# mapillary/OpenSfM

Hardware: AMD Instinct MI355X
Metric: image-pairs matched/sec (+ BA LM-iters/sec, 5k cams / 500k pts) (higher is better)
Workload: dtype i8 (exact int32 accumulate) + f64 RANSAC

## Files before the change

### opensfm_amd/csrc/ba.hip

```cpp
#ifdef OSFM_HIPEMU
#include <cassert>
#endif
#include <chrono>
#include <cmath>
#include <cstdio>
#include <cstring>
#include <numeric>
#include <vector>

#include <rocprim/rocprim.hpp>

#include "ba_math.h"
#include "osfm_internal.h"

using namespace osfm_ba;

namespace {

constexpr int kCoopObs = 256;

typedef double osfm_v2d __attribute__((ext_vector_type(2)));
__device__ __forceinline__ void st2(double *p, double a, double b) {
  osfm_v2d v;
  v.x = a;
// ... 126 lines not shown
    for (int m = 32; m >= 1; m >>= 1) v[k] += __shfl_xor(v[k], m);
  const int lane = threadIdx.x & 63, w = threadIdx.x >> 6;
  const int nw = (blockDim.x + 63) >> 6;
  if (nw == 1) return;
  if (lane == 0)
#pragma unroll
    for (int k = 0; k < NV; k++) lds[w * NV + k] = v[k];
  __syncthreads();
  if (threadIdx.x == 0)
#pragma unroll
    for (int k = 0; k < NV; k++) {
      double s = lds[k];
      for (int w2 = 1; w2 < nw; w2++) s += lds[w2 * NV + k];
      v[k] = s;
    }
}

template <int NV, int W, int N>
__device__ __forceinline__ void shot_sum(double (&v)[NV], double (&lds)[N] ) {
  static_assert(W == 1 || N >= W * NV, "shot_sum: lds is shorter than NV doubles per wavefront");
#ifdef OSFM_HIPEMU
  assert((int)blockDim.x == 64 * W);
#endif
#pragma unroll
  for (int i = 0; i < NV; i++)
#pragma unroll
    for (int m = 32; m >= 1; m >>= 1) v[i] += __shfl_xor(v[i], m);
  if (W == 1) return;
  const int lane = threadIdx.x & 63, w = threadIdx.x >> 6;
  if (lane == 0)
// ... 108 lines not shown
  double *qD;
  double *qE[2];
  double *qX;
  double *qXt;
  double *qx, *qy;
  int qT;
  double *qP, *qR, *qRn, *qC;
  double *zc;
  double *y;
  double *x, *r, *z, *p, *Ap, *b;
  double *scal;
  double *partial;
  double *partial2;
  double *dotp;
  double *rrp;
  int gen;
  GenDev g;
};

#define JA(o, c) d.Jpm[(long)(c) * d.M + (o)]
constexpr int kRowComps = 17;
constexpr int R_JP = 2, R_JR = 8, R_U = 14, R_V = 15, R_WT = 16;

__device__ __forceinline__ void row_jk(const Dev &d, long o, int s, double (&jk)[6]) {
  const int ci = d.shot_camera[s];
  const double u = JA(o, R_U), v = JA(o, R_V), wt = JA(o, R_WT), sg = d.o_sigma[o];
  const double *cam = d.cams + 3 * ci;
  const double k1 = cam[0], k2 = cam[1], f = cam[2];
  const bool other = d.cam_model && d.cam_model[ci] >= 2;
  double J[6];
// ... 186 lines not shown
__device__ __forceinline__ void up_residual(const Dev &d, int s, double r[3], double J[9]) {
  const double *R = d.shotR + 36 * (long)s, *u = d.up + 3 * (long)s;
  const double isd = 1.0 / d.up_sigma[s];
#pragma unroll
  for (int i = 0; i < 3; i++) {
    const double z = R[i] * u[0] + R[3 + i] * u[1] + R[6 + i] * u[2];
    r[i] = isd * (z - (i == 2 ? 1.0 : 0.0));
#pragma unroll
    for (int k = 0; k < 3; k++) {
      const double *dR = R + 9 + 9 * k;
      J[3 * i + k] = -isd * (dR[i] * u[0] + dR[3 + i] * u[1] + dR[6 + i] * u[2]);
    }
  }
}

__global__ void __launch_bounds__(1024) prior_cost_kernel(Dev d, const double *cams, const double *poses, const double *partial, long npart, double *out, double *absmax_slot, int jac) {
  __shared__ double lds[64];
  for (int c = 0; c < 2; c++) {
    double v[1] = {0.0};
    for (long i = threadIdx.x; i < npart; i += blockDim.x) v[0] += partial[i * 2 + c];
    block_sum<1, 1024>(v, lds);
    if (threadIdx.x == 0) out[c] = v[0];
    __syncthreads();
  }
  if (threadIdx.x == 0 && absmax_slot) *absmax_slot = 0.0;
  double v[1] = {0.0};
  for (int c = threadIdx.x; c < d.NC; c += blockDim.x) {
    if (d.cam_fixed[c]) continue;
    const double *q = cams + 3 * c, *pr = d.cam_prior + 3 * c, *sg = d.cam_sigma + 3 * c;
    const double e0 = (q[0] - pr[0]) / fmax(sg[0], kEps), e1 = (q[1] - pr[1]) / fmax(sg[1], kEps);
    const double e2 = log(q[2] / pr[2]) / fmax(sg[2], kEps);
    v[0] += 0.5 * (e0 * e0 + e1 * e1 + e2 * e2);
  }
  if (d.gps && d.gps_sigma)
    for (int s = threadIdx.x; s < d.S; s += blockDim.x) {
      const double sg = d.gps_sigma[s];
      const bool fixed = d.shot_fixed && d.shot_fixed[s];
      const double p3[3] = {poses[6 * s + 3], poses[6 * s + 4], poses[6 * s + 5]}, g3[3] = {d.gps[3 * s], d.gps[3 * s + 1], d.gps[3 * s + 2]};
      if (!(sg > 0) || fixed) continue;
      for (int i = 0; i < 3; i++) {
        const double e = (p3[i] - g3[i]) / sg;
        v[0] += 0.5 * e * e;
      }
    }
  if (d.up && d.up_sigma)
    for (int s = threadIdx.x; s < d.S; s += blockDim.x) {
      if (!(d.up_sigma[s] > 0) || (d.shot_fixed && d.shot_fixed[s])) continue;
      double r[3], J[9], rho, rho1;
      up_residual(d, s, r, J);
      loss_eval(OSFM_LOSS_CAUCHY, 1.0, r[0] * r[0] + r[1] * r[1] + r[2] * r[2], rho, rho1);
      v[0] += 0.5 * rho;
      if (jac) {
        const double wt = sqrt(rho1);
        for (int i = 0; i < 3; i++) d.up_r[3 * s + i] = wt * r[i];
        for (int i = 0; i < 9; i++) d.up_J[9 * s + i] = wt * J[i];
      }
    }
  block_sum<1, 1024>(v, lds);
  if (threadIdx.x == 0) out[0] += v[0];
}

template <int W>
__global__ void __launch_bounds__(64 * W) shot_grad_kernel(Dev d, const double *poses, int loss, double la) {
  __shared__ double red[W > 1 ? W * 36 : 1];
  const int s = (int)xcd_contiguous(blockIdx.x, gridDim.x), lane = threadIdx.x;
  const ShotFrame f = shot_frame(d, s);
  double v[36];
#pragma unroll
  for (int i = 0; i < 36; i++) v[i] = 0;
  for (long k = d.shot_off[s] + lane; k < d.shot_off[s + 1]; k += 64 * W) {
    double r[2], Jp[6], Jc[12], Jk[6];
    const int p = d.sm_point[k];
    project_obs<true>(f.model, d.pts + 3 * (long)p, f.pose, f.R, f.R + 9, f.cam, d.sm_x[k], d.sm_y[k], 1.0 / d.sm_sigma[k], r, Jp, Jc, Jk);
    double rho, rho1;
// ... 69 lines not shown
  const bool fixed = d.cam_fixed[c];
  const double *q = cams + 3 * c, *pr = d.cam_prior + 3 * c, *sg = d.cam_sigma + 3 * c;
  const double w0 = 1.0 / fmax(sg[0], kEps), w1 = 1.0 / fmax(sg[1], kEps), w2 = 1.0 / fmax(sg[2], kEps);
  const double e[3] = {(q[0] - pr[0]) * w0, (q[1] - pr[1]) * w1, log(q[2] / pr[2]) * w2};
  const double j[3] = {w0, w1, w2 / q[2]};
  const int dg[3] = {3, 5, 8};
  for (int k = 0; k < 3; k++) {
    const int i = d.cam0 + 3 * c + k;
    d.g_red[i] = fixed ? 0.0 : v[k] + j[k] * e[k];
    d.prior_diag[i] = fixed ? 0.0 : j[k] * j[k];
    d.diag_red[i] = fixed ? 0.0 : v[dg[k]] + j[k] * j[k];
  }
  for (int i = 0; i < 6; i++) d.Hcc[21 * (long)d.S + 6 * c + i] = v[3 + i];
}

constexpr int kCamRedT = 1024;
__global__ void __launch_bounds__(kCamRedT) cam_reduce_kernel(Dev d, int ncomp, const double *grad_cams) {
  __shared__ double lds[16 * 9];
  const int c = blockIdx.x;
  double v[9] = {0, 0, 0, 0, 0, 0, 0, 0, 0};
  for (int s0 = threadIdx.x; s0 < d.S; s0 += 4 * kCamRedT) {
    double p[4][9];
    bool on[4];
#pragma unroll
    for (int u = 0; u < 4; u++) {
      const int s = s0 + u * kCamRedT;
      const bool in = s < d.S;
      on[u] = in && d.shot_camera[in ? s : 0] == c;
#pragma unroll
      for (int i = 0; i < 9; i++) p[u][i] = (in && i < ncomp) ? d.part[9 * (long)s + i] : 0.0;
    }
#pragma unroll
    for (int u = 0; u < 4; u++)
      if (on[u])
#pragma unroll
        for (int i = 0; i < 9; i++) v[i] += p[u][i];
  }
  block_sum<9, kCamRedT>(v, lds);
  if (threadIdx.x == 0) {
    for (int i = 0; i < ncomp; i++) d.camred[9 * c + i] = v[i];
    if (grad_cams) cam_grad_one(d, grad_cams, c, v);
  }
}

__global__ void cam_grad_kernel(Dev d, const double *cams) {
  const int c = blockIdx.x * blockDim.x + threadIdx.x;
  if (c >= d.NC) return;
  double v[9];
  for (int i = 0; i < 9; i++) v[i] = d.camred[9 * c + i];
  cam_grad_one(d, cams, c, v);
}

__global__ void scale_init_kernel(Dev d) {
  const long i = (long)blockIdx.x * blockDim.x + threadIdx.x;
  if (i < d.nred) {
    bool fixed;
// ... 2291 lines not shown

__global__ void dot2_kernel(const double *a, const double *b, const double *c, const double *e, int n, double *o0, double *o1) {
  __shared__ double lds[32];
  double v[2] = {0, 0};
#pragma unroll 4
  for (int i = threadIdx.x; i < n; i += blockDim.x) {
    v[0] += a[i] * b[i];
    if (c) v[1] += c[i] * e[i];
  }
  block_sum<2, 1024>(v, lds);
  if (threadIdx.x == 0) {
    *o0 = v[0];
    if (c) *o1 = v[1];
  }
}
__global__ void pcg_init_kernel(const double *b, const double *z, double *x, double *r, double *p, int n, double *o_rz, double *o_bb, const double *sc, double *y) {
  __shared__ double lds[32];
  double v[2] = {0, 0};
#pragma unroll 4
  for (int i = threadIdx.x; i < n; i += blockDim.x) {
    const double bi = b[i], zi = z[i];
    x[i] = 0.0;
    r[i] = bi;
    p[i] = zi;
    y[i] = sc[i] * zi;
    v[0] += bi * zi;
    v[1] += bi * bi;
  }
  block_sum<2, 1024>(v, lds);
  if (threadIdx.x == 0) {
    *o_rz = v[0];
    *o_bb = v[1];
  }
}
__global__ void __launch_bounds__(TPB) pcg_step1_kernel(double *x, double *r, const double *p, const double *Ap, int n, const double *rz, const double *dot_part, int nparts,
                                                         double *o_pAp, double *rr_part, const double *sc = nullptr, double *y_out = nullptr) {
  __shared__ double lds[32];
  __shared__ double s_alpha;
  const int i = blockIdx.x * blockDim.x + threadIdx.x;
  {
    double pAp;
    if (dot_part) {
      double a[1] = {0.0};
      for (int q = threadIdx.x; q < nparts; q += TPB) a[0] += dot_part[q];
      block_sum<1, TPB>(a, lds);
      pAp = a[0];
    } else
// ... 29 lines not shown
  } else if (b < d.S + d.NC) {
    const int c = b - d.S;
    const double *Bi = d.Binv + 36 * (long)d.S + 9 * c, *rr = r + d.cam0 + 3 * c;
    for (int i = 0; i < 3; i++) z[d.cam0 + 3 * c + i] = Bi[3 * i] * rr[0] + Bi[3 * i + 1] * rr[1] + Bi[3 * i + 2] * rr[2];
  }
}
__global__ void pcg_step2_kernel(double *p, const double *z, int n, const double *rz_old, const double *rz_new, const double *sc, double *y) {
  const int i = blockIdx.x * blockDim.x + threadIdx.x;
  if (i >= n) return;
  const double beta = *rz_old != 0.0 ? *rz_new / *rz_old : 0.0;
  const double pi = z[i] + beta * p[i];
  p[i] = pi;
  y[i] = sc[i] * pi;
}

__global__ void __launch_bounds__(1024) candidate_kernel(Dev d, const double *y, const double *partial, long npart, double *out, const double *part2, long npart2,
                                                         double *out2, int do_rot) {
  __shared__ double lds[16 * 3];
  {
    double m[1] = {0.0};
    for (long i = threadIdx.x; i < npart; i += blockDim.x) m[0] += partial[i];
    block_sum<1, 1024>(m, lds);
    if (threadIdx.x == 0) out[0] = m[0];
    __syncthreads();
  }
  for (int c = 0; c < 2; c++) {
    double m[1] = {0.0};
    for (long i = threadIdx.x; i < npart2; i += blockDim.x) m[0] += part2[2 * i + c];
    block_sum<1, 1024>(m, lds);
    if (threadIdx.x == 0) out2[c] = m[0];
    __syncthreads();
  }
  double v[3] = {0, 0, 0};
  for (int c = threadIdx.x; c < d.NC; c += blockDim.x) {
    const double *q = d.cams + 3 * c;
    const bool fixed = d.cam_fixed[c];
    if (!fixed) {
      const double *pr = d.cam_prior + 3 * c, *sg = d.cam_sigma + 3 * c;
      const double wq[3] = {1.0 / fmax(sg[0], kEps), 1.0 / fmax(sg[1], kEps), 1.0 / fmax(sg[2], kEps)};
      const double e[3] = {(q[0] - pr[0]) * wq[0], (q[1] - pr[1]) * wq[1], log(q[2] / pr[2]) * wq[2]};
      const double j[3] = {wq[0], wq[1], wq[2] / q[2]};
      for (int k = 0; k < 3; k++) {
        const double m = j[k] * y[d.cam0 + 3 * c + k];
        v[0] -= m * (e[k] + 0.5 * m);
      }
    }
    for (int k = 0; k < 3; k++) {
      const double dl = fixed ? 0.0 : y[d.cam0 + 3 * c + k];
      d.cams_n[3 * c + k] = q[k] + dl;
      if (!fixed) {
        v[1] += dl * dl;
        v[2] += q[k] * q[k];
      }
    }
  }
  for (int s = threadIdx.x; s < d.S; s += blockDim.x) {
    const bool fixed = d.shot_fixed && d.shot_fixed[s];
    double ys[6], ps[6], g3[3] = {0, 0, 0}, sg = 0.0;
#pragma unroll
    for (int k = 0; k < 6; k++) {
      ys[k] = y[6 * s + k];
      ps[k] = d.poses[6 * s + k];
    }
    if (d.gps && d.gps_sigma) {
      sg = d.gps_sigma[s];
#pragma unroll
      for (int k = 0; k < 3; k++) g3[k] = d.gps[3 * s + k];
    }
    if (!fixed && sg > 0) {
      const double wq = 1.0 / sg;
      for (int k = 0; k < 3; k++) {
// ... 9 lines not shown
        v[0] -= m * (ru[i] + 0.5 * m);
      }
    }
    double pn[6];
    for (int k = 0; k < 6; k++) {
      const double dl = fixed ? 0.0 : ys[k];
      pn[k] = ps[k] + dl;
      d.poses_n[6 * s + k] = pn[k];
      if (!fixed) {
        v[1] += dl * dl;
        v[2] += ps[k] * ps[k];
      }
    }
    if (do_rot) rot_and_derivs(pn, d.shotR + 36 * (long)s, d.shotR + 36 * (long)s + 9);
  }
  block_sum<3, 1024>(v, lds);
  if (threadIdx.x == 0) {
    out[0] += v[0];
    out[1] = v[1];
    out[2] = v[2];
  }
}
__global__ void __launch_bounds__(TPB) candidate_points_kernel(Dev d, double *part) {
  __shared__ double lds[16];
  const long i = (long)blockIdx.x * TPB + threadIdx.x;
  double v[2] = {0, 0};
  if (i < 3L * d.P) {
    const bool fixed = d.point_fixed && d.point_fixed[i / 3];
    const double dl = fixed ? 0.0 : d.d_pt[i];
    d.pts_n[i] = d.pts[i] + dl;
    if (!fixed) {
      v[0] = dl * dl;
      v[1] = d.pts[i] * d.pts[i];
    }
  }
// ... 43 lines not shown
}
__global__ void reproj_kernel(Dev d, double *out) {
  const long o = (long)blockIdx.x * TPB + threadIdx.x;
  if (o >= d.M) return;
  const int s = d.o_shot[o], p = d.o_point[o];
  const double *R = d.shotR + 36 * (long)s;
  double r[2];
  const int cmodel = d.cam_model ? d.cam_model[d.shot_camera[s]] : 0;
  project_obs<false>(cmodel, d.pts + 3 * (long)p, d.poses + 6 * (long)s, R, R + 9,
                     cmodel >= 2 ? d.cam_ext + 16 * d.shot_camera[s] : d.cams + 3 * d.shot_camera[s], d.o_x[o], d.o_y[o],
                     1.0, r, nullptr, nullptr, nullptr);
  out[2 * o] = r[0];
  out[2 * o + 1] = r[1];
}

__global__ void border_dots_kernel(const double *Bc, const double *W, int nb, int n, double *out) {
  __shared__ double lds[32];
  const int i = blockIdx.x / nb, j = blockIdx.x % nb;
  double v[1] = {0.0};
#pragma unroll 4
  for (int t = threadIdx.x; t < n; t += blockDim.x) v[0] += Bc[(long)i * n + t] * W[(long)j * n + t];
  block_sum<1, 1024>(v, lds);
  if (threadIdx.x == 0) out[blockIdx.x] = v[0];
}
__global__ void border_rhs_kernel(const double *Bc, const double *SigInv, const double *r, double *z, int nb, int n, int cam0) {
  __shared__ double lds[32];
  __shared__ double y[8];
  for (int i = 0; i < nb; i++) {
    double v[1] = {0.0};
    for (int t = threadIdx.x; t < n; t += blockDim.x) v[0] += Bc[(long)i * n + t] * z[t];
    block_sum<1, 1024>(v, lds);
    if (threadIdx.x == 0) y[i] = r[cam0 + i] - v[0];
    __syncthreads();
  }
  if (threadIdx.x < nb) {
    double acc = 0.0;
    for (int j = 0; j < nb; j++) acc += SigInv[threadIdx.x * nb + j] * y[j];
    z[cam0 + threadIdx.x] = acc;
// ... 578 lines not shown
      }
      if (ctx->h_stage) {
        char *dst = (char *)ctx->h_stage + staged;
        memcpy(dst, h, bytes);
        staged += padded;
        e = hipMemcpyAsync(p, dst, bytes, hipMemcpyHostToDevice, st);
        return p;
      }
    }
    e = hipMemcpy(p, h, bytes, hipMemcpyHostToDevice);
    return p;
  }
};

inline int nblk(long n, int t = TPB) { return (int)std::max<long>(1, (n + t - 1) / t); }

struct BaSwitches {
  bool no_sband = getenv("OSFM_BA_NO_SBAND") != nullptr;
  bool check_band = getenv("OSFM_BA_CHECK_BAND") != nullptr;
  bool band_per_shot = getenv("OSFM_BA_BAND_PER_SHOT") != nullptr;
  bool wide_ldlt = getenv("OSFM_BA_WIDE_LDLT") != nullptr;
  const char *dense_cr_budget = getenv("OSFM_BA_DENSE_CR_BUDGET");
  bool gen_full_rows = getenv("OSFM_BA_GEN_FULL_ROWS") != nullptr;
  bool no_fast = getenv("OSFM_BA_NO_FAST") != nullptr;
  int fast_fail_at = getenv("OSFM_BA_FAST_FAIL_AT") ? atoi(getenv("OSFM_BA_FAST_FAIL_AT")) : -1;
  bool trace = getenv("OSFM_BA_TRACE") != nullptr;
  bool spin = getenv("OSFM_BA_NO_SPIN") == nullptr;
  double spin_us = getenv("OSFM_BA_SPIN_US") ? atof(getenv("OSFM_BA_SPIN_US")) : 2000.0;
};

// ... 156 lines not shown
    double *dh = (double *)dev_pinned;
    const int want = ++seq;
    hipLaunchKernelGGL(publish_kernel, dim3(1), dim3(64), 0, st, a, na, dh + ha_off, b, nb, (int *)(dh + 32) + hb_off, c, nc, dh + 34, (int *)(dh + 34 + nbr_), want);
    OSFM_HIP(hipGetLastError());
    const auto t0 = std::chrono::steady_clock::now();
    for (long it = 0; __atomic_load_n(hseq, __ATOMIC_ACQUIRE) != want; it++) {
      if ((it & 0x3FF) == 0x3FF && std::chrono::duration<double>(std::chrono::steady_clock::now() - t0).count() * 1e6 > spin_us) {
        OSFM_HIP(hipStreamSynchronize(st));
        OSFM_REQUIRE(__atomic_load_n(hseq, __ATOMIC_ACQUIRE) == want, OSFM_E_HIP, "the device never published round trip %d", want);
      }
    }
    return OSFM_OK;
  }

  void rot(const double *poses) { hipLaunchKernelGGL(shot_rot_kernel, dim3(nblk(d.S, 64)), dim3(64), 0, st, d, poses); }

  template <class F>
  void with_gen_model(F &&f) const {
    using std::integral_constant;
    if (d.g.NRr == 3) f(integral_constant<int, 3>{}, integral_constant<int, -1>{});
    else if (gen_uniform_model == OSFM_CAMERA_BROWN) f(integral_constant<int, 2>{}, integral_constant<int, OSFM_CAMERA_BROWN>{});
    else if (gen_uniform_model == OSFM_CAMERA_FISHEYE_OPENCV) f(integral_constant<int, 2>{}, integral_constant<int, OSFM_CAMERA_FISHEYE_OPENCV>{});
    else if (gen_uniform_model == OSFM_CAMERA_PERSPECTIVE) f(integral_constant<int, 2>{}, integral_constant<int, OSFM_CAMERA_PERSPECTIVE>{});
    else f(integral_constant<int, 2>{}, integral_constant<int, -1>{});
  }
  template <class F>
  void with_gen_kw(F &&f) const {
    using std::integral_constant;
    if (d.g.KW <= 4) f(integral_constant<int, 4>{});
    else if (d.g.KW <= 9) f(integral_constant<int, 9>{});
// ... 112 lines not shown
    if (!y_ready) hipLaunchKernelGGL(scale_vec_kernel, dim3(nblk(d.nred)), dim3(TPB), 0, sq, d.sc_red, x, d.y, d.nred);
    gen_rows_apply(0, sq);
    if (have_bpri && d.g.NB > 0) hipLaunchKernelGGL(gen_bpri_dot_kernel, dim3(d.g.NB, kBpriSlices), dim3(256), 0, sq, d, (const double *)d.y);
    hipLaunchKernelGGL(gen_schur_finish_kernel, dim3(nblk(d.nred)), dim3(TPB), 0, sq, d, x, (const double *)d.y, out, radius, 0, d.M > 0 ? 1 : 0,
                       have_bpri ? 1 : 0, dot_part);
  }

  void eval_enqueue(const double *cams, const double *poses, const double *pts, bool jac, bool rot_done = false) {
    if (d.gen) {
      const bool cand = poses == d.poses_n;
      return gen_eval_enqueue(cand ? d.g.cam_n : d.g.cam, cand ? d.g.bias_n : d.g.bias, cand ? d.g.rc_n : d.g.rc, poses, pts, jac);
    }
    if (!rot_done) rot(poses);
    if (jac) hipLaunchKernelGGL(eval_kernel<true>, dim3(d.nwg), dim3(kCoopObs), 0, st, d, cams, poses, pts, loss, loss_a);
    else hipLaunchKernelGGL(eval_kernel<false>, dim3(d.nwg), dim3(kCoopObs), 0, st, d, cams, poses, pts, loss, loss_a);
    hipLaunchKernelGGL(prior_cost_kernel, dim3(1), dim3(1024), 0, st, d, cams, poses, (const double *)d.partial, (long)d.nwg, d.scal + 8, d.scal + 10, jac ? 1 : 0);
  }
  int eval(const double *cams, const double *poses, const double *pts, bool jac, double *cost, double *sumsq) {
    eval_enqueue(cams, poses, pts, jac);
    OSFM_HIP(hipGetLastError());
    OSFM_TRY(fetch(d.scal + 8, 2, 0));
    *cost = hscal[0];
    if (sumsq) *sumsq = hscal[1];
    return OSFM_OK;
  }
  void gradients() {
    if (d.gen) return gen_gradients();
    if (shot_waves() > 1) hipLaunchKernelGGL(shot_grad_kernel<kShotWavesSmall>, dim3(d.S), dim3(64 * kShotWavesSmall), 0, st, d, (const double *)d.poses, loss, loss_a);
    else hipLaunchKernelGGL(shot_grad_kernel<1>, dim3(d.S), dim3(64), 0, st, d, (const double *)d.poses, loss, loss_a);
    if (!cams_inert) hipLaunchKernelGGL(cam_reduce_kernel, dim3(d.NC), dim3(kCamRedT), 0, st, d, 9, (const double *)d.cams);
    else hipLaunchKernelGGL(cam_grad_kernel, dim3(nblk(d.NC, 64)), dim3(64), 0, st, d, d.cams);
  }
  void bcr_solve_set(const RhsSet &rs) {
    if (use_sband) {
      hipLaunchKernelGGL(sband_solve_kernel, dim3((rs.nrhs + kSbSolveWaves - 1) / kSbSolveWaves), dim3(64 * kSbSolveWaves), sband_solve_lds(d.S, d.bw), st, d,
                         (const double *)sbL, rs, SbFuse{0, 0.0, nullptr, nullptr, nullptr, nullptr, nullptr, nullptr, nullptr});
      return;
    }
    const int N = d.ncl;
    const unsigned q = (unsigned)rs.nrhs;
    auto ne = [N](int s) { return (N + 2 * s - 1) / (2 * s); };
    int st0 = 2;
    while (ne(st0) > kMidWaves) st0 *= 2;
    hipLaunchKernelGGL(bcr_down_kernel, dim3(ne(1), q), dim3(64), 0, st, d, 1, rs, 1);
    for (int s = 2; s < st0; s *= 2) hipLaunchKernelGGL(bcr_down_kernel, dim3(ne(s), q), dim3(64), 0, st, d, s, rs, 0);
// ... 246 lines not shown
        if (shot_waves() > 1) hipLaunchKernelGGL((border_shot_kernel<3, kShotWavesSmall>), dim3(d.S), dim3(64 * kShotWavesSmall), 0, sx, d, wB, Bc, partB);
        else hipLaunchKernelGGL((border_shot_kernel<3, 1>), dim3(d.S), dim3(64), 0, sx, d, wB, Bc, partB);
        hipLaunchKernelGGL(border_cam_kernel<3>, dim3(d.NC), dim3(TPB), 0, sx, d, partB, dCm, radius);
      } else {
        hipLaunchKernelGGL(border_point_kernel<6>, dim3(d.nwg), dim3(kCoopObs), 0, sx, d, wB);
        if (shot_waves() > 1) hipLaunchKernelGGL((border_shot_kernel<6, kShotWavesSmall>), dim3(d.S), dim3(64 * kShotWavesSmall), 0, sx, d, wB, Bc, partB);
        else hipLaunchKernelGGL((border_shot_kernel<6, 1>), dim3(d.S), dim3(64), 0, sx, d, wB, Bc, partB);
        hipLaunchKernelGGL(border_cam_kernel<6>, dim3(d.NC), dim3(TPB), 0, sx, d, partB, dCm, radius);
      }
    }
    if (!pl.sband_fuse) rhs_enqueue(radius, sx);
    if (pl.side2) OSFM_HIP(hipEventRecord(ev_join, pl.side2));
    return OSFM_OK;
  }
  void border_sigma(int nb, int n6) {
    hipLaunchKernelGGL(border_dots_kernel, dim3(nb * nb), dim3(TPB), 0, st, Bc, Wb, nb, n6, dots);
    if (nb <= 6)
      hipLaunchKernelGGL(border_sigma_kernel, dim3(1), dim3(64), 0, st, dCm, dots, SigInv, nb, d_status + 1);
    else
      hipLaunchKernelGGL(gen_border_sigma_kernel, dim3(1), dim3(256), (size_t)nb * 2 * nb * sizeof(double), st, (const double *)dCm, (const double *)dots, SigInv, nb, d_status + 1);
  }
  int factorise_wide(const SolvePlan &pl) {
    if (pl.dense_cr) {
      OSFM_TRY(dbcr_factor(d_status));
    } else {
      hipLaunchKernelGGL(wide_tiles_kernel, dim3(d.wNB, d.wWb + 1), dim3(256), 0, st, d, d_status);
      const int ntile = d.wWb * (d.wWb + 1) / 2;
      for (int J = 0; J < d.wNB; J++) {
        const int left = std::min(d.wWb, d.wNB - 1 - J);
        hipLaunchKernelGGL(wide_factor_kernel, dim3(1 + (left == d.wWb ? ntile : left * (left + 1) / 2)), dim3(256), (size_t)2 * kWB * kWLd * sizeof(double), st, d, J, d_status);
      }
// ... 90 lines not shown
        if (d.g.NRr == 3) hipLaunchKernelGGL(gen_precond_shot_kernel<3>, dim3(d.S), dim3(64), 0, st, d, radius);
        else hipLaunchKernelGGL(gen_precond_shot_kernel<2>, dim3(d.S), dim3(64), 0, st, d, radius);
      }
    } else if (use_bcr && use_sband && !use_border && pl.all_cams_fixed && !z_solved) {
      if (sband_solved) {
        sband_solved = false;
        return;
      }
      hipLaunchKernelGGL(sband_solve_kernel, dim3(1), dim3(64 * kSbSolveWaves), sband_solve_lds(d.S, d.bw), st, d, (const double *)sbL,
                         RhsSet{d.b, 0, d.z, 0, 1, nullptr, nullptr, -1, 0}, SbFuse{1, radius, d.x, d.r, d.p, d.y, d.scal + 0, d.scal + 4, d.sc_red});
      return;
    } else if ((use_bcr || use_wide) && pl.all_cams_fixed) {
      hipLaunchKernelGGL(precond_cam_kernel, dim3(nblk(d.NC, 64)), dim3(64), 0, st, d, radius);
    } else if (!((use_bcr || use_wide) && use_border)) {
      hipLaunchKernelGGL(precond_shot_kernel, dim3(d.S), dim3(64), 0, st, d, radius);
      hipLaunchKernelGGL(cam_reduce_kernel, dim3(d.NC), dim3(kCamRedT), 0, st, d, 6, (const double *)nullptr);
      hipLaunchKernelGGL(precond_cam_kernel, dim3(nblk(d.NC, 64)), dim3(64), 0, st, d, radius);
    }
    precond(d.b, d.z, z_solved);
    z_solved = false;
    hipLaunchKernelGGL(pcg_init_kernel, dim3(1), dim3(1024), 0, st, d.b, d.z, d.x, d.r, d.p, d.nred, d.scal + 0, d.scal + 4, (const double *)d.sc_red, d.y);
  }
  int start_pcg(const SolvePlan &pl, double radius) {
    start_pcg_enqueue(pl, radius);
    return fetch(d.scal, 5, 0, d_status, (pl.try_bcr || pl.wide) ? 3 : 0, 0);
  }
  bool status_failed(const SolvePlan &pl) const { return (pl.try_bcr && hstat[0] != 0) || (use_wide && hstat[2] != 0) || (use_border && hstat[1] != 0); }
  void pcg_half(double radius, int rz_cur, bool leave_y = false) {
    matvec(d.p, d.Ap, radius, true, d.dotp);
    hipLaunchKernelGGL(pcg_step1_kernel, dim3(nbr_), dim3(TPB), 0, st, d.x, d.r, (const double *)d.p, (const double *)d.Ap, d.nred, (const double *)(d.scal + rz_cur),
                       (const double *)d.dotp, matvec_parts(), d.scal + 1, d.rrp, (const double *)d.sc_red, leave_y ? d.y : (double *)nullptr);
  }
  double residual_sq() const {
    double rr = 0.0;
    for (int q = 0; q < nbr_; q++) rr += hrr[(size_t)q];
    return rr;
// ... 45 lines not shown
    const int S = d.S, NP = d.P;
    if (!y_ready) hipLaunchKernelGGL(scale_vec_kernel, dim3(nbr_), dim3(TPB), 0, st, d.sc_red, d.x, d.y, d.nred);
    if (d.gen) {
      if (d.M > 0 && d.g.KW > 0) hipLaunchKernelGGL(gen_view_gather_kernel, dim3(nblk((long)d.g.NV * d.g.KW)), dim3(TPB), 0, st, d, (const double *)d.y);
      gen_schur_point(2, st);
      hipLaunchKernelGGL(finish_reduce_kernel, dim3(1), dim3(1024), 0, st, d.partial, (long)d.nwg, 1, d.scal + 16);
      hipLaunchKernelGGL(gen_candidate_kernel, dim3(1), dim3(1024), 0, st, d, (const double *)d.y, d.scal + 16);
      hipLaunchKernelGGL(gen_prior_kernel, dim3(nblk(gen_nprior(), kGenPriorTPB)), dim3(kGenPriorTPB), gen_prior_lds(2), st, d, (const double *)d.g.cam, (const double *)d.g.bias,
                         (const double *)d.g.rc, (const double *)d.poses, 2, (const double *)d.y, d.scal + 16);
      if (d.g.pt_prior_sigma && NP > 0) hipLaunchKernelGGL(gen_point_prior_kernel, dim3(nblk(NP)), dim3(TPB), 0, st, d, (const double *)d.pts, 2, d.scal + 16);
      hipLaunchKernelGGL(candidate_points_kernel, dim3(nblk(3L * NP)), dim3(TPB), 0, st, d, d.partial);
      hipLaunchKernelGGL(finish_reduce_kernel, dim3(1), dim3(1024), 0, st, d.partial, (long)nblk(3L * NP), 2, d.scal + 20);
    } else {
      hipLaunchKernelGGL(schur_point_coop_kernel<2>, dim3(d.nwg), dim3(kCoopObs), 0, st, d, d.y);
      hipLaunchKernelGGL(candidate_points_kernel, dim3(nblk(3L * NP)), dim3(TPB), 0, st, d, d.partial2);
      hipLaunchKernelGGL(candidate_kernel, dim3(1), dim3(1024), 0, st, d, (const double *)d.y, (const double *)d.partial, (long)d.nwg, d.scal + 16,
                         (const double *)d.partial2, (long)nblk(3L * NP), d.scal + 20, S <= 1024 ? 1 : 0);
    }
    swap_blocks();
    eval_enqueue(d.cams, d.poses, d.pts, true, !d.gen && S <= 1024);
    return prepare_enqueue();
  }
  int straight_line_step(const SolvePlan &pl, const osfm_ba_options *O, double radius, bool forced_failure, bool *done) {
    start_pcg_enqueue(pl, radius);
    pcg_half(radius, 0, true);
    OSFM_TRY(candidate_enqueue(true));
    OSFM_TRY(fetch(d.scal, 22, 0, d_status, 3, 0, d.rrp, nbr_));
    const double bb1 = hscal[4], rr = residual_sq();
    const double tol_first = std::max(O->pcg_tolerance, O->pcg_direct_tolerance);
    *done = !forced_failure && !status_failed(pl) && bb1 == bb1 && !std::isinf(bb1) && bb1 > 0 && rr == rr && rr <= tol_first * tol_first * bb1;
    if (!*done) OSFM_TRY(relinearise_old_point());
    return OSFM_OK;
  }
  int careful_step(const SolvePlan &pl, const osfm_ba_options *O, double radius, int iter, int *k, bool *bad, int64_t *pcg_total) {
    OSFM_TRY(start_pcg(pl, radius));
// ... 687 lines not shown
    while (pcur < NP) {
      int pe = pcur + 1;
      while (pe < NP && pe - pcur < kCoopObs && pt_off[(size_t)pe + 1] - pt_off[(size_t)pcur] <= kCoopObs) pe++;
      wg_pt.push_back(pe);
      pcur = pe;
    }
    if (wg_pt.size() < 2) wg_pt.push_back(0);
    d.nwg = (int)wg_pt.size() - 1;
    d.wg_pt = A.upload(wg_pt.data(), wg_pt.size(), e);
  }
  pl.bp_keys = bp_keys;
  pl.bp_pts = bp_pts;
  return OSFM_OK;
}

static void alloc_work_vectors(Arena &A, hipError_t &e, Solver &sv, int nbord) {
  Dev &d = sv.d;
  GenDev &g = d.g;
  const bool gen = d.gen != 0;
  const int S = d.S, NP = d.P, NC = d.NC;
  const long M = d.M;
  d.shotR = A.alloc<double>((size_t)36 * S, e);
  d.Jpm = A.alloc<double>((size_t)(gen ? g.ncomp : kRowComps) * M, e);
  d.sm_wt = A.alloc<double>((size_t)std::max<long>(1, M), e);
  {
    int *ss = A.alloc<int>((size_t)M, e), *sp = A.alloc<int>((size_t)M, e);
    double *sx = A.alloc<double>((size_t)M, e), *sy = A.alloc<double>((size_t)M, e), *ssg = A.alloc<double>((size_t)M, e);
    if (e == hipSuccess && M > 0)
      hipLaunchKernelGGL(gather_sm_kernel, dim3(nblk(M)), dim3(TPB), 0, sv.st, d.shot_obs, d.o_shot, d.o_point, d.o_x, d.o_y, d.o_sigma, M, ss,
                         sp, sx, sy, ssg);
// ... 22 lines not shown
  d.camred = A.alloc<double>((size_t)9 * NC, e);
  d.zc = A.alloc<double>(nr, e);
  d.y = A.alloc<double>(nr, e);
  d.x = A.alloc<double>(nr, e);
  d.r = A.alloc<double>(nr, e);
  d.z = A.alloc<double>(nr, e);
  d.p = A.alloc<double>(nr, e);
  d.Ap = A.alloc<double>(nr, e);
  d.b = A.alloc<double>(nr, e);
  d.scal = A.alloc<double>(32, e);
  const long nbmax = std::max<long>(std::max<long>(nblk(M), nblk(3L * NP)), d.nwg);
  d.partial = A.alloc<double>((size_t)2 * nbmax + 16, e);
  d.partial2 = A.alloc<double>((size_t)2 * nblk(3L * NP) + 16, e);
  d.dotp = A.alloc<double>((size_t)nblk(d.nred) + NC + 16, e);
  d.rrp = A.alloc<double>((size_t)nblk(d.nred) + 16, e);
}

static int choose_band_solver(osfm_ctx *ctx, const osfm_ba_options *O, Arena &A, hipError_t &e, Solver &sv, SolvePlan &pl) {
  Dev &d = sv.d;
  GenDev &g = d.g;
  const BaSwitches &sw = sv.sw;
  const bool gen = d.gen != 0;
  const int S = d.S, NP = d.P;
  const long M = d.M;
  constexpr int kLdsBw = 10;
  static_assert(kLdsBw <= kSbMaxBw, "the one-workgroup band factor runs on the LDS clusters' bands");
  pl.wide = O->preconditioner == 0 && S >= 2 && pl.bw_true > kLdsBw && pl.bw_true <= kWMaxBw;
  d.bw = O->preconditioner == 1 ? 0 : (pl.wide ? pl.bw_true : std::min(pl.bw_true, kMaxBw));
  if (S < 2) d.bw = 0;
  const int band_nslice = (d.bw + 1 + kBandSlice - 1) / kBandSlice;
// ... 234 lines not shown
  d.S = S; d.P = NP; d.NC = NC; d.M = M;
  d.cam0 = 6 * S;
  d.gen = gen ? 1 : 0;
  if (gen) OSFM_TRY(gen_border_layout(P, G, A, e, sv));
  plan.nbord = gen ? d.g.NB : 3 * NC;
  d.nred = 6 * S + plan.nbord;
  OSFM_TRY(upload_blocks(P, G, A, e, d));
  OSFM_TRY(build_observation_orders(P, G, A, e, sv, plan));
  alloc_work_vectors(A, e, sv, plan.nbord);
  OSFM_TRY(choose_band_solver(ctx, O, A, e, sv, plan));
  OSFM_TRY(plan_border_and_iteration(P, O, G, A, e, sv, plan));
  sv.d_status = A.alloc<int>(4, e);
  sv.d_reproj = (gen ? G->reproj3 != nullptr : P->reproj_err != nullptr) ? A.alloc<double>((size_t)(gen ? 3 : 2) * M, e) : nullptr;
  OSFM_REQUIRE(e == hipSuccess, OSFM_E_NOMEM, "BA device allocation/upload failed: %s", hipGetErrorString(e));
  OSFM_HIP(hipMemsetAsync(d.scal, 0, 32 * sizeof(double), sv.st));
  OSFM_TRY(sv.pinned(nblk(d.nred)));
  OSFM_HIP(hipStreamSynchronize(sv.st));

  const auto t_run = std::chrono::steady_clock::now();
  double cost = 0, sumsq = 0, radius = 0;
  OSFM_TRY(sv.eval(d.cams, d.poses, d.pts, true, &cost, &sumsq));
  Rp->initial_cost = cost;
  Rp->seconds_setup = std::chrono::duration<double>(t_run - t_start).count();
  Rp->rmse_normalized_initial = std::sqrt(sumsq / (double)rmse_rows);
  Rp->cost_history[0] = cost;
  OSFM_TRY(sv.mark("first evaluation"));
  const SolvePlan &pl = plan;
  OSFM_TRY(sv.lm_loop(pl, O, Rp, &cost, &sumsq, &radius));
  OSFM_HIP(hipStreamSynchronize(sv.st));

// ... 20 lines not shown
```

Before: 2.768 million.

## Spread single-workgroup BA reductions across many workgroups with last-block ticket finish

Several bundle-adjustment kernels that ran as one 1024-thread workgroup (prior cost, candidate, PCG init, camera reduce, border dots) now run over many TPB workgroups. Each writes per-block partials, and the last block, chosen by an atomic ticket counter with release/acquire fences, does the final reduction. The aim is to remove the serial single-CU bottleneck on these per-iteration reductions. It also drops the S<=1024 limit so rotation updates are always fused into the candidate kernel. The cost is extra scratch buffers, atomics and fences, plus a ticket scheme that depends on counters resetting correctly between launches.

```diff
diff --git a/opensfm_amd/csrc/ba.hip b/opensfm_amd/csrc/ba.hip
--- a/opensfm_amd/csrc/ba.hip
+++ b/opensfm_amd/csrc/ba.hip
@@ -164,6 +164,36 @@
       for (int w2 = 1; w2 < nw; w2++) s += lds[w2 * NV + k];
       v[k] = s;
     }
+}
+
+constexpr int kTicketStride = 32;
+enum { TK_INIT = 0, TK_CAND, TK_PRIOR, TK_DOTS, TK_CAM };
+constexpr int kSpreadWgs = 64;
+__device__ __forceinline__ void vm_drain() {
+#if defined(__HIP_DEVICE_COMPILE__)
+  asm volatile("s_waitcnt vmcnt(0)" ::: "memory");
+#endif
+}
+__device__ __forceinline__ bool last_workgroup(unsigned *counter, unsigned total, int &flag) {
+  if (total == 1u) {
+    __syncthreads();
+    return true;
+  }
+  vm_drain();
+  __syncthreads();
+  if (threadIdx.x == 0) {
+    __builtin_amdgcn_fence(__ATOMIC_RELEASE, "agent");
+    vm_drain();
+    const unsigned t = atomicAdd(counter, 1u);
+    flag = t == total - 1u;
+    if (flag) {
+      atomicAdd(counter, 0u - total);
+      __builtin_amdgcn_fence(__ATOMIC_ACQUIRE, "agent");
+      vm_drain();
+    }
+  }
+  __syncthreads();
+  return flag != 0;
 }
 
 template <int NV, int W, int N>
@@ -302,6 +332,8 @@
   double *partial2;
   double *dotp;
   double *rrp;
+  double *sh_init, *sh_cand, *sh_prior, *sh_cam, *sh_dots;
+  unsigned *tickets;
   int gen;
   GenDev g;
 };
@@ -518,18 +550,17 @@
   }
 }
 
-__global__ void __launch_bounds__(1024) prior_cost_kernel(Dev d, const double *cams, const double *poses, const double *partial, long npart, double *out, double *absmax_slot, int jac) {
-  __shared__ double lds[64];
-  for (int c = 0; c < 2; c++) {
-    double v[1] = {0.0};
-    for (long i = threadIdx.x; i < npart; i += blockDim.x) v[0] += partial[i * 2 + c];
-    block_sum<1, 1024>(v, lds);
-    if (threadIdx.x == 0) out[c] = v[0];
-    __syncthreads();
-  }
-  if (threadIdx.x == 0 && absmax_slot) *absmax_slot = 0.0;
+__global__ void __launch_bounds__(TPB) prior_cost_kernel(Dev d, const double *cams, const double *poses, const double *partial, long npart, double *out, double *absmax_slot, int jac) {
+  __shared__ double lds[4 * 3];
+  __shared__ int last;
+  const int gt = blockIdx.x * TPB + threadIdx.x, gs = gridDim.x * TPB;
+  double m[2] = {0, 0};
+  for (long i = gt; i < npart; i += gs) {
+    m[0] += partial[2 * i];
+    m[1] += partial[2 * i + 1];
+  }
   double v[1] = {0.0};
-  for (int c = threadIdx.x; c < d.NC; c += blockDim.x) {
+  for (int c = gt; c < d.NC; c += gs) {
     if (d.cam_fixed[c]) continue;
     const double *q = cams + 3 * c, *pr = d.cam_prior + 3 * c, *sg = d.cam_sigma + 3 * c;
     const double e0 = (q[0] - pr[0]) / fmax(sg[0], kEps), e1 = (q[1] - pr[1]) / fmax(sg[1], kEps);
@@ -537,7 +568,7 @@
     v[0] += 0.5 * (e0 * e0 + e1 * e1 + e2 * e2);
   }
   if (d.gps && d.gps_sigma)
-    for (int s = threadIdx.x; s < d.S; s += blockDim.x) {
+    for (int s = gt; s < d.S; s += gs) {
       const double sg = d.gps_sigma[s];
       const bool fixed = d.shot_fixed && d.shot_fixed[s];
       const double p3[3] = {poses[6 * s + 3], poses[6 * s + 4], poses[6 * s + 5]}, g3[3] = {d.gps[3 * s], d.gps[3 * s + 1], d.gps[3 * s + 2]};
@@ -548,7 +579,7 @@
       }
     }
   if (d.up && d.up_sigma)
-    for (int s = threadIdx.x; s < d.S; s += blockDim.x) {
+    for (int s = gt; s < d.S; s += gs) {
       if (!(d.up_sigma[s] > 0) || (d.shot_fixed && d.shot_fixed[s])) continue;
       double r[3], J[9], rho, rho1;
       up_residual(d, s, r, J);
@@ -560,8 +591,22 @@
         for (int i = 0; i < 9; i++) d.up_J[9 * s + i] = wt * J[i];
       }
     }
-  block_sum<1, 1024>(v, lds);
-  if (threadIdx.x == 0) out[0] += v[0];
+  double w[3] = {m[0], m[1], v[0]};
+  block_sum<3, TPB>(w, lds);
+  if (threadIdx.x == 0)
+#pragma unroll
+    for (int k = 0; k < 3; k++) d.sh_prior[3 * blockIdx.x + k] = w[k];
+  if (!last_workgroup(d.tickets + TK_PRIOR * kTicketStride, gridDim.x, last)) return;
+  double t[3] = {0, 0, 0};
+  for (int q = threadIdx.x; q < (int)gridDim.x; q += TPB)
+#pragma unroll
+    for (int k = 0; k < 3; k++) t[k] += d.sh_prior[3 * q + k];
+  block_sum<3, TPB>(t, lds);
+  if (threadIdx.x == 0) {
+    out[0] = t[0] + t[2];
+    out[1] = t[1];
+    if (absmax_slot) *absmax_slot = 0.0;
+  }
 }
 
 template <int W>
@@ -661,32 +706,39 @@
   for (int i = 0; i < 6; i++) d.Hcc[21 * (long)d.S + 6 * c + i] = v[3 + i];
 }
 
-constexpr int kCamRedT = 1024;
-__global__ void __launch_bounds__(kCamRedT) cam_reduce_kernel(Dev d, int ncomp, const double *grad_cams) {
-  __shared__ double lds[16 * 9];
-  const int c = blockIdx.x;
+constexpr int kCamSlices = 32;
+__global__ void __launch_bounds__(TPB) cam_reduce_kernel(Dev d, int ncomp, const double *grad_cams) {
+  __shared__ double lds[4 * 9];
+  __shared__ int last;
+  const int c = blockIdx.x, K = gridDim.y;
   double v[9] = {0, 0, 0, 0, 0, 0, 0, 0, 0};
-  for (int s0 = threadIdx.x; s0 < d.S; s0 += 4 * kCamRedT) {
-    double p[4][9];
-    bool on[4];
-#pragma unroll
-    for (int u = 0; u < 4; u++) {
-      const int s = s0 + u * kCamRedT;
-      const bool in = s < d.S;
-      on[u] = in && d.shot_camera[in ? s : 0] == c;
-#pragma unroll
-      for (int i = 0; i < 9; i++) p[u][i] = (in && i < ncomp) ? d.part[9 * (long)s + i] : 0.0;
-    }
-#pragma unroll
-    for (int u = 0; u < 4; u++)
-      if (on[u])
-#pragma unroll
-        for (int i = 0; i < 9; i++) v[i] += p[u][i];
-  }
-  block_sum<9, kCamRedT>(v, lds);
+  for (int s = blockIdx.y * TPB + threadIdx.x; s < d.S; s += K * TPB) {
+    double p[9];
+    const bool on = d.shot_camera[s] == c;
+#pragma unroll
+    for (int i = 0; i < 9; i++) p[i] = i < ncomp ? d.part[9 * (long)s + i] : 0.0;
+    if (on)
+#pragma unroll
+      for (int i = 0; i < 9; i++) v[i] += p[i];
+  }
+  block_sum<9, TPB>(v, lds);
+  double *share = d.sh_cam + 9 * (long)c * kCamSlices;
+  if (threadIdx.x == 0)
+#pragma unroll
+    for (int i = 0; i < 9; i++) share[9 * blockIdx.y + i] = v[i];
+  if (!last_workgroup(d.tickets + (TK_CAM + c) * kTicketStride, K, last)) return;
+  if (threadIdx.x < 9) {
+    double s = 0.0;
+    for (int k = 0; k < K; k++) s += share[9 * k + threadIdx.x];
+    lds[threadIdx.x] = s;
+  }
+  __syncthreads();
   if (threadIdx.x == 0) {
-    for (int i = 0; i < ncomp; i++) d.camred[9 * c + i] = v[i];
-    if (grad_cams) cam_grad_one(d, grad_cams, c, v);
+    double t[9];
+#pragma unroll
+    for (int i = 0; i < 9; i++) t[i] = lds[i];
+    for (int i = 0; i < ncomp; i++) d.camred[9 * c + i] = t[i];
+    if (grad_cams) cam_grad_one(d, grad_cams, c, t);
   }
 }
 
@@ -3008,23 +3060,36 @@
     if (c) *o1 = v[1];
   }
 }
-__global__ void pcg_init_kernel(const double *b, const double *z, double *x, double *r, double *p, int n, double *o_rz, double *o_bb, const double *sc, double *y) {
-  __shared__ double lds[32];
+__global__ void __launch_bounds__(TPB) pcg_init_kernel(const double *b, const double *z, double *x, double *r, double *p, int n, double *o_rz, double *o_bb, const double *sc,
+                                                        double *y, double *share, unsigned *ticket) {
+  __shared__ double lds[8];
+  __shared__ int last;
+  const int i = blockIdx.x * TPB + threadIdx.x;
   double v[2] = {0, 0};
-#pragma unroll 4
-  for (int i = threadIdx.x; i < n; i += blockDim.x) {
+  if (i < n) {
     const double bi = b[i], zi = z[i];
     x[i] = 0.0;
     r[i] = bi;
     p[i] = zi;
     y[i] = sc[i] * zi;
-    v[0] += bi * zi;
-    v[1] += bi * bi;
-  }
-  block_sum<2, 1024>(v, lds);
+    v[0] = bi * zi;
+    v[1] = bi * bi;
+  }
+  block_sum<2, TPB>(v, lds);
   if (threadIdx.x == 0) {
-    *o_rz = v[0];
-    *o_bb = v[1];
+    share[2 * blockIdx.x] = v[0];
+    share[2 * blockIdx.x + 1] = v[1];
+  }
+  if (!last_workgroup(ticket, gridDim.x, last)) return;
+  double t[2] = {0, 0};
+  for (int q = threadIdx.x; q < (int)gridDim.x; q += TPB) {
+    t[0] += share[2 * q];
+    t[1] += share[2 * q + 1];
+  }
+  block_sum<2, TPB>(t, lds);
+  if (threadIdx.x == 0) {
+    *o_rz = t[0];
+    *o_bb = t[1];
   }
 }
 __global__ void __launch_bounds__(TPB) pcg_step1_kernel(double *x, double *r, const double *p, const double *Ap, int n, const double *rz, const double *dot_part, int nparts,
@@ -3084,25 +3149,19 @@
   y[i] = sc[i] * pi;
 }
 
-__global__ void __launch_bounds__(1024) candidate_kernel(Dev d, const double *y, const double *partial, long npart, double *out, const double *part2, long npart2,
-                                                         double *out2, int do_rot) {
-  __shared__ double lds[16 * 3];
-  {
-    double m[1] = {0.0};
-    for (long i = threadIdx.x; i < npart; i += blockDim.x) m[0] += partial[i];
-    block_sum<1, 1024>(m, lds);
-    if (threadIdx.x == 0) out[0] = m[0];
-    __syncthreads();
-  }
-  for (int c = 0; c < 2; c++) {
-    double m[1] = {0.0};
-    for (long i = threadIdx.x; i < npart2; i += blockDim.x) m[0] += part2[2 * i + c];
-    block_sum<1, 1024>(m, lds);
-    if (threadIdx.x == 0) out2[c] = m[0];
-    __syncthreads();
+__global__ void __launch_bounds__(TPB) candidate_kernel(Dev d, const double *y, const double *partial, long npart, double *out, const double *part2, long npart2,
+                                                        double *out2, int do_rot) {
+  __shared__ double lds[4 * 6];
+  __shared__ int last;
+  const int gt = blockIdx.x * TPB + threadIdx.x, gs = gridDim.x * TPB;
+  double m[3] = {0, 0, 0};
+  for (long i = gt; i < npart; i += gs) m[0] += partial[i];
+  for (long i = gt; i < npart2; i += gs) {
+    m[1] += part2[2 * i];
+    m[2] += part2[2 * i + 1];
   }
   double v[3] = {0, 0, 0};
-  for (int c = threadIdx.x; c < d.NC; c += blockDim.x) {
+  for (int c = gt; c < d.NC; c += gs) {
     const double *q = d.cams + 3 * c;
     const bool fixed = d.cam_fixed[c];
     if (!fixed) {
@@ -3124,7 +3183,7 @@
       }
     }
   }
-  for (int s = threadIdx.x; s < d.S; s += blockDim.x) {
+  for (int s = gt; s < d.S; s += gs) {
     const bool fixed = d.shot_fixed && d.shot_fixed[s];
     double ys[6], ps[6], g3[3] = {0, 0, 0}, sg = 0.0;
 #pragma unroll
@@ -3164,11 +3223,23 @@
     }
     if (do_rot) rot_and_derivs(pn, d.shotR + 36 * (long)s, d.shotR + 36 * (long)s + 9);
   }
-  block_sum<3, 1024>(v, lds);
+  double w[6] = {m[0], m[1], m[2], v[0], v[1], v[2]};
+  block_sum<6, TPB>(w, lds);
+  if (threadIdx.x == 0)
+#pragma unroll
+    for (int k = 0; k < 6; k++) d.sh_cand[6 * blockIdx.x + k] = w[k];
+  if (!last_workgroup(d.tickets + TK_CAND * kTicketStride, gridDim.x, last)) return;
+  double t[6] = {0, 0, 0, 0, 0, 0};
+  for (int q = threadIdx.x; q < (int)gridDim.x; q += TPB)
+#pragma unroll
+    for (int k = 0; k < 6; k++) t[k] += d.sh_cand[6 * q + k];
+  block_sum<6, TPB>(t, lds);
   if (threadIdx.x == 0) {
-    out[0] += v[0];
-    out[1] = v[1];
-    out[2] = v[2];
+    out[0] = t[0] + t[3];
+    out[1] = t[4];
+    out[2] = t[5];
+    out2[0] = t[1];
+    out2[1] = t[2];
   }
 }
 __global__ void __launch_bounds__(TPB) candidate_points_kernel(Dev d, double *part) {
@@ -3242,14 +3313,22 @@
   out[2 * o + 1] = r[1];
 }
 
-__global__ void border_dots_kernel(const double *Bc, const double *W, int nb, int n, double *out) {
-  __shared__ double lds[32];
-  const int i = blockIdx.x / nb, j = blockIdx.x % nb;
+constexpr int kDotSlices = 32;
+__global__ void __launch_bounds__(TPB) border_dots_kernel(const double *Bc, const double *W, int nb, int n, double *out, double *share, unsigned *ticket) {
+  __shared__ double lds[4];
+  __shared__ int last;
+  const int i = blockIdx.x / nb, j = blockIdx.x % nb, K = gridDim.y;
   double v[1] = {0.0};
 #pragma unroll 4
-  for (int t = threadIdx.x; t < n; t += blockDim.x) v[0] += Bc[(long)i * n + t] * W[(long)j * n + t];
-  block_sum<1, 1024>(v, lds);
-  if (threadIdx.x == 0) out[blockIdx.x] = v[0];
+  for (int t = blockIdx.y * TPB + threadIdx.x; t < n; t += K * TPB) v[0] += Bc[(long)i * n + t] * W[(long)j * n + t];
+  block_sum<1, TPB>(v, lds);
+  if (threadIdx.x == 0) share[blockIdx.x * K + blockIdx.y] = v[0];
+  if (!last_workgroup(ticket, gridDim.x * gridDim.y, last)) return;
+  for (int e = threadIdx.x; e < nb * nb; e += TPB) {
+    double s = 0.0;
+    for (int k = 0; k < K; k++) s += share[e * K + k];
+    out[e] = s;
+  }
 }
 __global__ void border_rhs_kernel(const double *Bc, const double *SigInv, const double *r, double *z, int nb, int n, int cam0) {
   __shared__ double lds[32];
@@ -3858,6 +3937,7 @@
 };
 
 inline int nblk(long n, int t = TPB) { return (int)std::max<long>(1, (n + t - 1) / t); }
+inline int spread_grid(long n_elem, long n_part) { return std::max(nblk(n_elem), (int)std::min<long>(kSpreadWgs, nblk(n_part))); }
 
 struct BaSwitches {
   bool no_sband = getenv("OSFM_BA_NO_SBAND") != nullptr;
@@ -4044,6 +4124,7 @@
   }
 
   void rot(const double *poses) { hipLaunchKernelGGL(shot_rot_kernel, dim3(nblk(d.S, 64)), dim3(64), 0, st, d, poses); }
+  int cam_slices() const { return std::min(kCamSlices, nblk(d.S)); }
 
   template <class F>
   void with_gen_model(F &&f) const {
@@ -4186,7 +4267,8 @@
     if (!rot_done) rot(poses);
     if (jac) hipLaunchKernelGGL(eval_kernel<true>, dim3(d.nwg), dim3(kCoopObs), 0, st, d, cams, poses, pts, loss, loss_a);
     else hipLaunchKernelGGL(eval_kernel<false>, dim3(d.nwg), dim3(kCoopObs), 0, st, d, cams, poses, pts, loss, loss_a);
-    hipLaunchKernelGGL(prior_cost_kernel, dim3(1), dim3(1024), 0, st, d, cams, poses, (const double *)d.partial, (long)d.nwg, d.scal + 8, d.scal + 10, jac ? 1 : 0);
+    hipLaunchKernelGGL(prior_cost_kernel, dim3(spread_grid(std::max(d.S, d.NC), d.nwg)), dim3(TPB), 0, st, d, cams, poses, (const double *)d.partial, (long)d.nwg, d.scal + 8,
+                       d.scal + 10, jac ? 1 : 0);
   }
   int eval(const double *cams, const double *poses, const double *pts, bool jac, double *cost, double *sumsq) {
     eval_enqueue(cams, poses, pts, jac);
@@ -4200,7 +4282,7 @@
     if (d.gen) return gen_gradients();
     if (shot_waves() > 1) hipLaunchKernelGGL(shot_grad_kernel<kShotWavesSmall>, dim3(d.S), dim3(64 * kShotWavesSmall), 0, st, d, (const double *)d.poses, loss, loss_a);
     else hipLaunchKernelGGL(shot_grad_kernel<1>, dim3(d.S), dim3(64), 0, st, d, (const double *)d.poses, loss, loss_a);
-    if (!cams_inert) hipLaunchKernelGGL(cam_reduce_kernel, dim3(d.NC), dim3(kCamRedT), 0, st, d, 9, (const double *)d.cams);
+    if (!cams_inert) hipLaunchKernelGGL(cam_reduce_kernel, dim3(d.NC, cam_slices()), dim3(TPB), 0, st, d, 9, (const double *)d.cams);
     else hipLaunchKernelGGL(cam_grad_kernel, dim3(nblk(d.NC, 64)), dim3(64), 0, st, d, d.cams);
   }
   void bcr_solve_set(const RhsSet &rs) {
@@ -4477,7 +4559,8 @@
     return OSFM_OK;
   }
   void border_sigma(int nb, int n6) {
-    hipLaunchKernelGGL(border_dots_kernel, dim3(nb * nb), dim3(TPB), 0, st, Bc, Wb, nb, n6, dots);
+    const int slices = std::max(1, std::min(std::min(kDotSlices, nblk(n6, 8 * TPB)), 256 / (nb * nb)));
+    hipLaunchKernelGGL(border_dots_kernel, dim3(nb * nb, slices), dim3(TPB), 0, st, Bc, Wb, nb, n6, dots, d.sh_dots, d.tickets + TK_DOTS * kTicketStride);
     if (nb <= 6)
       hipLaunchKernelGGL(border_sigma_kernel, dim3(1), dim3(64), 0, st, dCm, dots, SigInv, nb, d_status + 1);
     else
@@ -4598,12 +4681,13 @@
       hipLaunchKernelGGL(precond_cam_kernel, dim3(nblk(d.NC, 64)), dim3(64), 0, st, d, radius);
     } else if (!((use_bcr || use_wide) && use_border)) {
       hipLaunchKernelGGL(precond_shot_kernel, dim3(d.S), dim3(64), 0, st, d, radius);
-      hipLaunchKernelGGL(cam_reduce_kernel, dim3(d.NC), dim3(kCamRedT), 0, st, d, 6, (const double *)nullptr);
+      hipLaunchKernelGGL(cam_reduce_kernel, dim3(d.NC, cam_slices()), dim3(TPB), 0, st, d, 6, (const double *)nullptr);
       hipLaunchKernelGGL(precond_cam_kernel, dim3(nblk(d.NC, 64)), dim3(64), 0, st, d, radius);
     }
     precond(d.b, d.z, z_solved);
     z_solved = false;
-    hipLaunchKernelGGL(pcg_init_kernel, dim3(1), dim3(1024), 0, st, d.b, d.z, d.x, d.r, d.p, d.nred, d.scal + 0, d.scal + 4, (const double *)d.sc_red, d.y);
+    hipLaunchKernelGGL(pcg_init_kernel, dim3(nbr_), dim3(TPB), 0, st, d.b, d.z, d.x, d.r, d.p, d.nred, d.scal + 0, d.scal + 4, (const double *)d.sc_red, d.y, d.sh_init,
+                       d.tickets + TK_INIT * kTicketStride);
   }
   int start_pcg(const SolvePlan &pl, double radius) {
     start_pcg_enqueue(pl, radius);
@@ -4679,11 +4763,11 @@
     } else {
       hipLaunchKernelGGL(schur_point_coop_kernel<2>, dim3(d.nwg), dim3(kCoopObs), 0, st, d, d.y);
       hipLaunchKernelGGL(candidate_points_kernel, dim3(nblk(3L * NP)), dim3(TPB), 0, st, d, d.partial2);
-      hipLaunchKernelGGL(candidate_kernel, dim3(1), dim3(1024), 0, st, d, (const double *)d.y, (const double *)d.partial, (long)d.nwg, d.scal + 16,
-                         (const double *)d.partial2, (long)nblk(3L * NP), d.scal + 20, S <= 1024 ? 1 : 0);
+      hipLaunchKernelGGL(candidate_kernel, dim3(spread_grid(std::max(S, d.NC), d.nwg)), dim3(TPB), 0, st, d, (const double *)d.y, (const double *)d.partial, (long)d.nwg,
+                         d.scal + 16, (const double *)d.partial2, (long)nblk(3L * NP), d.scal + 20, 1);
     }
     swap_blocks();
-    eval_enqueue(d.cams, d.poses, d.pts, true, !d.gen && S <= 1024);
+    eval_enqueue(d.cams, d.poses, d.pts, true, !d.gen);
     return prepare_enqueue();
   }
   int straight_line_step(const SolvePlan &pl, const osfm_ba_options *O, double radius, bool forced_failure, bool *done) {
@@ -5401,6 +5485,7 @@
   return OSFM_OK;
 }
 
+inline size_t ticket_words(int NC) { return (size_t)(TK_CAM + std::max(1, NC)) * kTicketStride; }
 static void alloc_work_vectors(Arena &A, hipError_t &e, Solver &sv, int nbord) {
   Dev &d = sv.d;
   GenDev &g = d.g;
@@ -5453,6 +5538,13 @@
   d.partial2 = A.alloc<double>((size_t)2 * nblk(3L * NP) + 16, e);
   d.dotp = A.alloc<double>((size_t)nblk(d.nred) + NC + 16, e);
   d.rrp = A.alloc<double>((size_t)nblk(d.nred) + 16, e);
+  const size_t nspread = (size_t)std::max(nblk(std::max(S, NC)), kSpreadWgs);
+  d.sh_init = A.alloc<double>((size_t)2 * nblk(d.nred), e);
+  d.sh_cand = A.alloc<double>(6 * nspread, e);
+  d.sh_prior = A.alloc<double>(3 * nspread, e);
+  d.sh_cam = A.alloc<double>((size_t)9 * kCamSlices * std::max(1, NC), e);
+  d.sh_dots = A.alloc<double>((size_t)std::max(1, nbord * nbord) * kDotSlices, e);
+  d.tickets = A.alloc<unsigned>(ticket_words(NC), e);
 }
 
 static int choose_band_solver(osfm_ctx *ctx, const osfm_ba_options *O, Arena &A, hipError_t &e, Solver &sv, SolvePlan &pl) {
@@ -5717,6 +5809,7 @@
   sv.d_reproj = (gen ? G->reproj3 != nullptr : P->reproj_err != nullptr) ? A.alloc<double>((size_t)(gen ? 3 : 2) * M, e) : nullptr;
   OSFM_REQUIRE(e == hipSuccess, OSFM_E_NOMEM, "BA device allocation/upload failed: %s", hipGetErrorString(e));
   OSFM_HIP(hipMemsetAsync(d.scal, 0, 32 * sizeof(double), sv.st));
+  OSFM_HIP(hipMemsetAsync(d.tickets, 0, ticket_words(NC) * sizeof(unsigned), sv.st));
   OSFM_TRY(sv.pinned(nblk(d.nred)));
   OSFM_HIP(hipStreamSynchronize(sv.st));
 
```

Result: no change. 2.767 million (-0.0%).
